# synsin0/StreamingFlow

Hardware: AMD Instinct MI355X
Metric: ODE-steps/s on 200x200x64 BEV (GRU-ODE future-state path, full FuturePredictionODE.forward) (higher is better)
Workload: dtype f32; 1 GPU; BASELINE config 2: C=64, BEV 200x200 (latent 50x50), timeset 'shipped' (8 observations, 7 targets), variable-step euler: 10 ODE steps + 8 jumps per sample, 32 sample(s) per forward per GPU; batch_per_gpu=32, parallelism=replicas x1 (sample sharding; no data-path collective)

## Files before the change

streamingflow_amd/csrc/conv_wino.hip:

```cpp
#include "sf_math.h"
#include "sf_launch.h"

#include <cstdlib>
#include <type_traits>

namespace sf {

#ifdef SF_STAMP
static __device__ unsigned long long* g_sf_stamps = nullptr;
hipError_t set_stamp_buffer_wino(unsigned long long* p) { return hipMemcpyToSymbol(HIP_SYMBOL(g_sf_stamps), &p, sizeof(p)); }
#else
hipError_t set_stamp_buffer_wino(unsigned long long*) { return hipErrorNotSupported; }
#endif

constexpr int WN_THREADS = 512;
constexpr long SF_WINO_SPLIT_WGS_DEFAULT = 512;
typedef __attribute__((address_space(3))) void wn_lds_void;

__device__ __forceinline__ f32x4 wn_lds_read128(const float* p) {
  typedef const __attribute__((address_space(3))) f32x4 lds_f4;
  return *(lds_f4*)p;
}
__device__ __forceinline__ void wn_barrier() {
  asm volatile("" ::: "memory");
// ... 139 lines not shown
  float* const Pbuf = Vbuf + G::NVB * G::V_FLOATS;
  float* const Park = Pbuf + G::NPB * G::P_FLOATS;
  float* const SBuf = Park + G::PARK;
  float* const SCbuf = SBuf + G::SB;
  float* const PVbuf = SCbuf + G::SC;
  (void)PVbuf;
  int lin_ = (int)blockIdx.x;
  const int pi_ = (int)__umulhi((unsigned)lin_, L.wn_m[0]);
  lin_ -= pi_ * L.wg_base[1];
  const ConvProblem& P = L.p[0];
  const ConvProblem& PX = L.p[pi_];
  const int tid = threadIdx.x, lane = tid & 63;
  const int wave = __builtin_amdgcn_readfirstlane(tid >> 6);
  const int H = P.Hout, W = P.Wout;
  const WnAxis ax(DIL ? W : 2, DIL ? P.dil : 1), ay(DIL ? H : 2, DIL ? P.dil : 1);
  const int tiles_x = DIL ? ax.nt : (W + 1) >> 1;
  const int tpi = tiles_x;
  const int nbx = ((CAT ? P.n_img * tiles_x : tiles_x) + TW - 1) / TW, nby = (L.wn_nty + TH - 1) / TH;
  const int ncb = P.cout_pad / COUT_T;
  const int nblk = nbx * nby * (CAT ? 1 : P.n_img), per_xcd = (nblk + 7) >> 3;
  const int lin = lin_, xcd = lin & 7, slot_ = lin >> 3;
#if SF_W5_MAGIC
  auto mdiv = [](const int nn, const unsigned m) { return m ? (int)__umulhi((unsigned)nn, m) : nn; };
  const unsigned m_ncb = L.wn_m[1], m_nbx = L.wn_m[2], m_nby = L.wn_m[3], m_tpi = L.wn_m[4];
  (void)m_tpi;
  const int tb_ = mdiv(slot_, m_ncb);
  int b = xcd * per_xcd + tb_;
  if (b >= nblk) return;
  const int bq_ = mdiv(b, m_nbx);
  const int bx = b - bq_ * nbx; b = bq_;
  const int bi_ = mdiv(b, m_nby);
  const int by = b - bi_ * nby;
  const int img = CAT ? mdiv(bx * TW, m_tpi) : bi_;
#else
  const int tb_ = slot_ / ncb;
  int b = xcd * per_xcd + tb_;
  if (b >= nblk) return;
  const int bx = b % nbx; b /= nbx;
  const int by = b % nby;
  const int img = CAT ? (bx * TW) / tpi : b / nby;
#endif
  const int ct0 = CAT ? bx * TW - img * tpi : 0;
  const int cn0 = CAT ? (tpi - ct0 < TW ? tpi - ct0 : TW) : TW;
  const int ty0 = L.wn_ty0 + by * TH, tx0 = CAT ? ct0 : bx * TW;
  int px0 = 0, pt0 = 0, py0 = 0, qt0 = 0;
  if constexpr (DIL) { ax.decode(tx0, px0, pt0); ay.decode(ty0, py0, qt0); }
  SF_STAMP_AT(L, 0);
#ifdef SF_STAMP
  SF_STAMP_VAL(L, 8, (unsigned long long)__builtin_amdgcn_s_getreg((31 << 11) | 4));
  SF_STAMP_VAL(L, 9, (unsigned long long)__builtin_amdgcn_s_getreg((31 << 11) | 20));
  SF_STAMP_VAL(L, 10, (unsigned long long)nkc_stamp(P));
#endif
  const int cout0 = (slot_ - tb_ * ncb) * COUT_T;
  const int nkc_g = P.cin_pad >> 4;
  const int nkc = GRP * nkc_g;
  const int NS = nkc * 4;
  const int c0 = P.c0;
  const int img_px_i = P.Hin * P.Win;
  const int up = DIL ? 0 : P.in_up;
  const int Win = P.Win;
#if defined(__HIP_DEVICE_COMPILE__)
  auto make_rsrc = [](const float* base, size_t bytes) {
    const unsigned nrec = bytes < 0x7fffffffull ? (unsigned)bytes : 0x7fffffffu;
    return __builtin_amdgcn_make_buffer_rsrc(const_cast<float*>(base), (short)0, (int)nrec, 0x00020000);
  };
  const size_t img_px = (size_t)P.Hin * P.Win;
  const size_t n_in = (CAT && img + 1 < P.n_img) ? 2 : 1;
  const __amdgpu_buffer_rsrc_t rsrc0 = make_rsrc(PX.in0 + (size_t)img * img_px * P.in0_cs, n_in * img_px * P.in0_cs * sizeof(float));
  const __amdgpu_buffer_rsrc_t rsrc1 = make_rsrc(PX.in1 ? PX.in1 + (size_t)img * img_px * P.in1_cs : PX.in0, PX.in1 ? n_in * img_px * P.in1_cs * sizeof(float) : 0);
  const __amdgpu_buffer_rsrc_t rsrc_u = make_rsrc(PX.w_wino, (size_t)nkc * 16 * P.cout_pad * 16 * sizeof(float));
#endif
  constexpr bool SCALED = G::SC > 0 && (EPI == EPI_AFFINE || EPI == EPI_SAMPLE);
  const bool scaled = SCALED && PX.in_scale != nullptr;
  typedef __attribute__((address_space(3))) int lds_int;
  float* const TabF = Park + 512;
  auto tab = [&](const int i) -> int { return *(const lds_int*)(TabF + i); };
  if constexpr (DIL) {
    if (tid < 72) {
      int v = 0;
      if (tid < PW) { int ix; v = ax.patch_coord(tid, px0, pt0, TW, W, ix) ? ix : -1; }
      else if (tid >= 32 && tid < 32 + G::PH) { int iy; v = ay.patch_coord(tid - 32, py0, qt0, TH, H, iy) ? iy : -1; }
      else if (tid >= 48 && tid < 60) {
        const bool isx = tid < 56;
        const int t = isx ? tx0 + (tid - 48) : ty0 + (tid - 56);
        const WnAxis& a = isx ? ax : ay;
        int pp, tt;
        a.decode(t, pp, tt);
        v = (t < a.nt && pp < P.dil) ? pp + P.dil * 2 * tt : (isx ? W : H);
      } else if (tid >= 60) {
        const bool isx = tid < 68;
        const int t = isx ? tx0 + (tid - 60) : ty0 + (tid - 68);
        int pp, tt;
        (isx ? ax : ay).decode(t, pp, tt);
        const int r = pp - (isx ? px0 : py0), lim = isx ? G::RX : G::RY;
        v = r < lim ? r : lim - 1;
      }
      *(lds_int*)(TabF + tid) = v;
    }
    asm volatile("s_waitcnt lgkmcnt(0)" ::: "memory");
    wn_barrier();
  }
  SF_STAMP_AT(L, 14);
  int pv0[NP], pv1[DIL ? 1 : NP];
  int piy[GRP > 1 ? NP : 1], pix_[GRP > 1 ? NP : 1];
  int pvs0[GRP > 1 ? NP : 1], pvs1[GRP > 1 ? NP : 1];
  (void)piy; (void)pix_; (void)pvs0; (void)pvs1;
  const int npw = G::ND / 8 + (wave < G::ND % 8 ? 1 : 0);
#pragma unroll
  for (int d = 0; d < NP; ++d) {
    const int e = (d * 8 + wave) * 64 + lane;
    const int pix = e >> 2, quad = e & 3;
    const int py = pix / PW, px = pix - py * PW;
    int iy = 2 * ty0 - 1 + py, ix = 2 * tx0 - 1 + px;
    int run = 0;
    if constexpr (CAT) {
      run = px >= 2 * cn0 + 2 ? 1 : 0;
      ix = run ? px - (2 * cn0 + 2) - 1 : ix;
    }
    bool ok = pix < G::NPX && (unsigned)iy < (unsigned)H && (unsigned)ix < (unsigned)W && (!CAT || (img + run < P.n_img && (run == 0 || cn0 < TW)));
    if constexpr (DIL) {
      const int pyc = py < G::PH ? py : 0;
      ix = tab(px); iy = tab(32 + pyc);
      ok = pix < G::NPX && ix >= 0 && iy >= 0;
    }
    const int pofs = DIL ? iy * W + ix : (iy >> up) * Win + (ix >> up) + (CAT ? run * img_px_i : 0);
    if constexpr (GRP > 1) {
      const bool in_blk = pix < G::NPX && (!CAT || (img + run < P.n_img && (run == 0 || cn0 < TW)));
      piy[d] = in_blk ? iy : -(1 << 20);
      pix_[d] = ix;
      pv0[d] = (pofs * P.in0_cs + quad * 4) * 4;
      pv1[d] = (pofs * P.in1_cs + quad * 4) * 4;
    } else {
      pv0[d] = ok ? (pofs * P.in0_cs + quad * 4) * 4 : (int)0x80000000;
      if constexpr (!DIL) pv1[d] = ok ? (pofs * P.in1_cs + quad * 4) * 4 : (int)0x80000000;
    }
  }
  int g_kc = 0, g_grp = 0;
  constexpr bool CAT_SC = CAT && G::PV == 0 && G::SC > 0;
  int run_bits = 0;
  if constexpr (CAT_SC) {
#pragma unroll
    for (int d = 0; d < NP; ++d) {
      const int pix = ((d * 8 + wave) * 64 + lane) >> 2;
      run_bits |= ((pix - (pix / PW) * PW) >= 2 * cn0 + 2 ? 1 : 0) << d;
    }
  }
  (void)run_bits;
  (void)g_kc; (void)g_grp;
  SF_STAMP_AT(L, 15);
  if constexpr (G::PV > 0) {
    static_assert(G::PV == 0 || NP == 1, "one piece per wave");
    *(lds_int*)(PVbuf + tid) = pv0[0];
    *(lds_int*)(PVbuf + 512 + tid) = pv1[0];
    asm volatile("s_waitcnt lgkmcnt(0)" ::: "memory");
  }
  auto issue_patch = [&](const int kc) {
    float* const dst = Pbuf + (G::NPB == 2 ? (kc & 1) : 0) * G::P_FLOATS;
    const bool from1 = !DIL && kc * 16 >= c0;
#if defined(__HIP_DEVICE_COMPILE__)
    if constexpr (GRP > 1) {
      if (g_kc == 0) {
        const int ga = (g_grp * 11) >> 5, gb = g_grp - 3 * ga;
        const int sy = 3 * ga - 3, sx = 3 * gb - 3;
        const int dlt = (sy * Win + sx) * 4;
#pragma unroll
        for (int d = 0; d < NP; ++d) {
          const bool okg = (unsigned)(piy[d] + sy) < (unsigned)H && (unsigned)(pix_[d] + sx) < (unsigned)W;
          pvs0[d] = okg ? pv0[d] + dlt * P.in0_cs : (int)0x80000000;
          pvs1[d] = okg ? pv1[d] + dlt * P.in1_cs : (int)0x80000000;
        }
      }
      const bool f1 = g_kc * 16 >= c0;
      const int so = f1 ? (g_kc * 16 - c0) * 4 : g_kc * 64;
#pragma unroll
      for (int d = 0; d < NP; ++d) {
        if (d >= npw) continue;
        float* const dB = dst + (d * 8 + wave) * 256;
        if (f1) {
          asm volatile("; patch from in1");
          __builtin_amdgcn_raw_ptr_buffer_load_lds(rsrc1, (wn_lds_void*)dB, 16, pvs1[d], so, 0, 0);
        } else {
          asm volatile("; patch from in0");
          __builtin_amdgcn_raw_ptr_buffer_load_lds(rsrc0, (wn_lds_void*)dB, 16, pvs0[d], so, 0, 0);
        }
      }
      if (++g_kc == nkc_g) { g_kc = 0; ++g_grp; }
      (void)kc; (void)from1;
      return;
    }
    if constexpr (G::PV > 0) {
      if (npw > 0) {
        int pv;
        asm volatile("ds_read_b32 %0, %1\n\ts_waitcnt lgkmcnt(0)" : "=v"(pv) : "v"((int)(size_t)(lds_int*)(PVbuf + (from1 ? 512 : 0) + tid)) : "memory");
        float* const dB = dst + wave * 256;
        if (from1) __builtin_amdgcn_raw_ptr_buffer_load_lds(rsrc1, (wn_lds_void*)dB, 16, pv, (kc * 16 - c0) * 4, 0, 0);
        else __builtin_amdgcn_raw_ptr_buffer_load_lds(rsrc0, (wn_lds_void*)dB, 16, pv, kc * 64, 0, 0);
      }
      return;
    }
#pragma unroll
    for (int d = 0; d < NP; ++d) {
      if (d >= npw) continue;
      float* const dB = dst + (d * 8 + wave) * 256;
      if constexpr (DIL) {
        __builtin_amdgcn_raw_ptr_buffer_load_lds(rsrc0, (wn_lds_void*)dB, 16, pv0[d], kc * 64, 0, 0);
      } else {
        if (from1) {
          asm volatile("; patch from in1");
          __builtin_amdgcn_raw_ptr_buffer_load_lds(rsrc1, (wn_lds_void*)dB, 16, pv1[d], (kc * 16 - c0) * 4, 0, 0);
        } else {
          asm volatile("; patch from in0");
          __builtin_amdgcn_raw_ptr_buffer_load_lds(rsrc0, (wn_lds_void*)dB, 16, pv0[d], kc * 64, 0, 0);
        }
      }
    }
#else
    (void)dst; (void)from1;
#endif
  };
  auto scale_patch = [&](const int kc) {
    if constexpr (SCALED) {
      if (scaled && kc * 16 < c0) {
// ... 45 lines not shown
                       : ((2 * tyl) * PW + 2 * txl + ((CAT && txl >= cn0) ? 2 : 0)) * 16 + quad * 4;
    const float* const a = src + tp + r1 * PW * 16;
    const float* const bb = src + tp + r2 * PW * 16;
    float* const o = dst + ((ih * 4) * WT + wt) * 16 + ((quad ^ ((wt >> 2) & 2)) << 2);
    typedef __attribute__((address_space(3))) f32x4 lds_f4w;
    const f32x4 w0 = wn_lds_read128(a) + sg * wn_lds_read128(bb);
    const f32x4 w2 = wn_lds_read128(a + 32) + sg * wn_lds_read128(bb + 32);
    *(lds_f4w*)(o) = wn5_sub4(w0, w2);
    const f32x4 w1 = wn_lds_read128(a + 16) + sg * wn_lds_read128(bb + 16);
    *(lds_f4w*)(o + WT * 16) = w1 + w2;
    *(lds_f4w*)(o + 2 * WT * 16) = wn5_sub4(w2, w1);
    const f32x4 w3 = wn_lds_read128(a + 48) + sg * wn_lds_read128(bb + 48);
    *(lds_f4w*)(o + 3 * WT * 16) = wn5_sub4(w1, w3);
  };
  float scv = 1.f;
  if constexpr (SCALED)
    if (scaled && tid < c0) scv = PX.in_scale[(size_t)img * c0 + tid];
    if (CAT_SC && scaled && tid >= c0 && tid < 2 * c0 && img + 1 < P.n_img) scv = PX.in_scale[(size_t)(img + 1) * c0 + (tid - c0)];
  issue_patch(0);
  f32x4 A[2][2];
  A[0][0] = load_A(0, 0); A[0][1] = load_A(0, 1);
  A[1][0] = load_A(1, 0); A[1][1] = load_A(1, 1);
  float sbv = tid < COUT_T ? 1.f : 0.f;
  if (tid < 2 * COUT_T) {
    const int co = cout0 + (tid < COUT_T ? tid : tid - COUT_T);
    if (co < P.cout) {
      if (tid < COUT_T) { if (PX.scale) sbv = PX.scale[co]; }
      else if (PX.bias) sbv = PX.bias[(P.bias_per_img ? (size_t)img * P.cout : 0) + co];
    }
  }
  SF_STAMP_AT(L, 11);
  wn_wait(4);
  if constexpr (SCALED) {
    if (scaled) {
      if (tid < G::SC) SCbuf[tid] = scv;
      asm volatile("s_waitcnt lgkmcnt(0)" ::: "memory");
      wn_barrier();
      scale_patch(0);
      asm volatile("s_waitcnt lgkmcnt(0)" ::: "memory");
    }
  }
  wn_barrier();
  SF_STAMP_AT(L, 12);
  transform(0);
  SF_STAMP_AT(L, 13);
  if (tid < 2 * COUT_T) SBuf[tid] = sbv;
  if (!MODE_A) issue_patch(1);
  asm volatile("s_waitcnt lgkmcnt(0)" ::: "memory");
  wn_barrier();
  SF_STAMP_AT(L, 1);

  f32x4 acc[4][2][NB];
  int b_cur = b_off;
  auto step = [&](const int kc, auto p_c, auto first_c) {
    constexpr int p = decltype(p_c)::value, slot = p & 1;
    constexpr bool first = decltype(first_c)::value;
    const float* const vb = Vbuf + (G::NVB == 2 ? (kc & 1) : 0) * G::V_FLOATS + p * WT * 16 + b_cur;
    f32x4 Bf[NB];
#pragma unroll
    for (int nb = 0; nb < NB; ++nb) Bf[nb] = wn_lds_read128(vb + nb * 256);
    __builtin_amdgcn_sched_barrier(0);
#pragma unroll
    for (int mb = 0; mb < 2; ++mb) {
#pragma unroll
      for (int e = 0; e < 4; ++e)
#pragma unroll
        for (int nb = 0; nb < NB; ++nb) {
          const f32x4 cin = (first && e == 0) ? (f32x4){0.f, 0.f, 0.f, 0.f} : acc[p][mb][nb];
          if (SF_W5_ABL & 16) acc[p][mb][nb] = (e == 0 && nb == 0 && mb == 0) ? cin + A[slot][mb] * Bf[nb] : cin;
          else acc[p][mb][nb] = __builtin_amdgcn_mfma_f32_16x16x4f32(A[slot][mb][e], Bf[nb][e], cin, 0, 0, 0);
        }
      __builtin_amdgcn_sched_barrier(0);
      if (!(SF_W5_ABL & 4)) A[slot][mb] = load_A(kc * 4 + p + 2, mb);
      __builtin_amdgcn_sched_barrier(0);
    }
  };
  auto chunk = [&](const int kc, auto first_c, auto more_c) {
    constexpr bool more = decltype(more_c)::value;
    if (MODE_A && more && !(SF_W5_ABL & 2)) issue_patch(kc + 1);
    step(kc, std::integral_constant<int, 0>{}, first_c);
    step(kc, std::integral_constant<int, 1>{}, first_c);
    if (MODE_A && more) {
      wn_wait(4);
      scale_patch(kc + 1);
      asm volatile("s_waitcnt lgkmcnt(0)" ::: "memory");
      if (!(SF_W5_ABL & 8)) wn_barrier();
      if (!(SF_W5_ABL & 1)) transform(kc + 1);
    }
    step(kc, std::integral_constant<int, 2>{}, first_c);
    step(kc, std::integral_constant<int, 3>{}, first_c);
    if (more) {
      if constexpr (MODE_A) {
        asm volatile("s_waitcnt lgkmcnt(0)" ::: "memory");
        if (!(SF_W5_ABL & 8)) wn_barrier();
      } else {
        wn_wait(4);
        wn_barrier();
        transform(kc + 1);
        if (kc + 2 < nkc) issue_patch(kc + 2);
        asm volatile("s_waitcnt lgkmcnt(0)" ::: "memory");
        wn_barrier();
      }
    }
  };
  chunk(0, std::true_type{}, std::true_type{});
  for (int kc = 1; kc + 1 < nkc; ++kc) chunk(kc, std::false_type{}, std::true_type{});
  if constexpr (WT == 16) {
    int t2 = tid;
    asm volatile("" : "+v"(t2));
    const int j2 = t2 & 15, g2 = (t2 & 63) >> 4;
    b_cur = (ih * 4 * WT + j2) * 16 + ((g2 ^ ((j2 >> 2) & 2)) << 2);
  }
  chunk(nkc - 1, std::false_type{}, std::false_type{});
  SF_STAMP_AT(L, 2);

  if (SF_W5_ABL & 32) {
    f32x4 sacc = (f32x4){0.f, 0.f, 0.f, 0.f};
#pragma unroll
    for (int p = 0; p < 4; ++p)
#pragma unroll
      for (int mb = 0; mb < 2; ++mb)
#pragma unroll
        for (int nb = 0; nb < NB; ++nb) sacc += acc[p][mb][nb];
    if (sacc[0] + sacc[1] + sacc[2] + sacc[3] == 1.2345f) PX.out[tid] = sacc[0];
    return;
  }
  float* const Tb = Vbuf;
  wn_barrier();
  int tid_e = tid;
  if constexpr (WT == 16) asm volatile("" : "+v"(tid_e));
  {
    typedef __attribute__((address_space(3))) f32x4 lds_f4w;
    const int j = tid_e & 15, g = (tid_e & 63) >> 4;
    const int tw_base = ((ih * 2) * WT + j) * 64;
#pragma unroll
    for (int mb = 0; mb < 2; ++mb) {
      const int tw = tw_base + (((hh * 8 + mb * 4 + g) ^ j) << 2);
#pragma unroll
      for (int nb = 0; nb < NB; ++nb) {
        const f32x4 m0 = acc[0][mb][nb], m1 = acc[1][mb][nb], m2 = acc[2][mb][nb], m3 = acc[3][mb][nb];
        *(lds_f4w*)(Tb + tw + nb * 16 * 64) = (m0 + m1) + m2;
        *(lds_f4w*)(Tb + tw + nb * 16 * 64 + WT * 64) = wn5_sub4(m1, m2 + m3);
      }
    }
  }
  const int cq = tid_e & 15, wt_e = WT == 32 ? tid_e >> 4 : (tid_e >> 4) & (WT - 1);
  const bool has_tile = WT == 32 || tid_e < 16 * WT;
  const int tyl_e = wt_e >> 3, txl_e = wt_e & 7;
  const bool run_e = CAT && txl_e >= cn0;
  const int ty = ty0 + tyl_e, tx = run_e ? txl_e - cn0 : tx0 + txl_e;
  int oy0 = 2 * ty, ox0 = 2 * tx, ostep = 1;
  if constexpr (DIL) {
    ostep = P.dil;
    ox0 = tab(48 + txl_e);
    oy0 = tab(56 + tyl_e);
  }
  constexpr bool affine = EPI == EPI_AFFINE, lng = EPI == EPI_LNG, smp = EPI == EPI_SAMPLE;
  const float* const t_a = (affine || lng) ? PX.add : PX.e0;
  const float* const t_b = PX.e1;
  const int cs_a = (affine || lng) ? P.add_cs : P.e0_cs, cs_b = P.e1_cs;
  const bool img_ok = has_tile && (!CAT || img + (run_e ? 1 : 0) < P.n_img);
  const bool x0 = img_ok && ox0 < W, x1 = img_ok && ox0 + ostep < W, y0ok = oy0 < H, y1ok = oy0 + ostep < H;
  const unsigned pix = (x0 && y0ok) ? (unsigned)(oy0 * W + ox0 + (run_e ? H * W : 0)) : 0u;
  const int cl = cq * 4;
  const int c = cout0 + cl;
  const bool c_ok = c < P.cout;
// ... 232 lines not shown
}
bool wino_takes(const ConvProblem& q, int epi) {
  if (epi == EPI_LNG) return wino_takes_ln7(q);
  if (epi == EPI_SAMPLE) {
    static const int on = [] { const char* v = std::getenv("SF_WINO_SAMPLE"); return v ? std::atoi(v) : 1; }();
    const double img_px = (double)q.Hin * q.Win;
    if (!on || q.dil != 1 || q.in_up || q.add || q.add_scale || q.pool2 || q.add_up || q.bias_per_img || q.scale || (q.cout % 8) || (q.c1 != 0) ||
        2.0 * 4.0 * img_px * q.cout >= 2147483648.0 || (!q.e0 && !q.philox))
      return false;
    return wino_takes(q, EPI_AFFINE);
  }
  if (epi != EPI_AFFINE && epi != EPI_BLEND) return false;
  if (!q.w_wino || q.KH != 3 || q.KW != 3 || q.stride != 1 || q.dil < 1 || q.pad != q.dil || (q.in_up && q.dil != 1) || q.gather || q.gate || q.se_sum ||
      (q.in_scale && (epi != EPI_AFFINE || q.dil != 1 || q.c0 > 256)) ||
      q.nsplit > 1 || q.chansum || q.acc_in || q.fuse_w || q.out_planar || (epi == EPI_AFFINE && (q.mode & 4)))
    return false;
  if (q.pool2 && (epi != EPI_AFFINE || q.dil != 1 || q.out2 || (q.Hout & 1) || (q.Wout & 1))) return false;
  if (q.add_up && (epi != EPI_AFFINE || q.dil != 1 || !q.add || (q.Hout & 1) || (q.Wout & 1))) return false;
  if ((q.c0 % 16) || (q.c1 % 16) || q.c0 + q.c1 != q.cin_pad || (q.cout_pad % 64) || (q.cout % 4)) return false;
  if (q.Hout != (q.Hin << q.in_up) || q.Wout != (q.Win << q.in_up) || q.Hout < 16 || q.Wout < 32) return false;
  if (q.dil > 1 && (q.c1 != 0 || epi != EPI_AFFINE || q.Hout / q.dil < 5 || q.Wout / q.dil < 5)) return false;
  const double img_bytes = 4.0 * q.Hin * q.Win;
  if (img_bytes * q.out_cs >= 2147483648.0 || img_bytes * q.add_cs >= 2147483648.0 || img_bytes * q.e0_cs >= 2147483648.0 ||
      img_bytes * q.e1_cs >= 2147483648.0 || img_bytes * q.out2_cs >= 2147483648.0)
    return false;
  if (img_bytes * q.in0_cs >= 2147483648.0 || img_bytes * q.in1_cs >= 2147483648.0 || 4.0 * 16 * q.cout_pad * q.cin_pad >= 2147483648.0) return false;
  return true;
}

static bool wino_cat(const ConvProblem& q) {
  static const int on = [] { const char* v = std::getenv("SF_WINO_CAT"); return v ? std::atoi(v) : 1; }();
  const int tpi = (q.Wout + 1) / 2;
  static const int cat_scaled = [] { const char* v = std::getenv("SF_WINO_CAT_SCALED"); return v ? std::atoi(v) : 1; }();
  if (!on || q.dil != 1 || q.in_up || q.n_img < 2 || tpi < 8 || q.bias_per_img || ((q.in_scale || q.add_scale) && !cat_scaled)) return false;
  const int plain = (tpi + 7) / 8 * 8;
  if (plain * 100 < tpi * 110) {
    if (q.cout_pad < 128 || plain * 100 < tpi * 104) return false;
    const char* const v = std::getenv("SF_WINO_CAT_WIDE");
    if (v && std::atoi(v) == 0) return false;
  }
  const double img_bytes = 4.0 * q.Hin * q.Win;
  const int cs = q.in0_cs > q.in1_cs ? q.in0_cs : q.in1_cs;
  const int co = q.out_cs > q.add_cs ? q.out_cs : q.add_cs;
  const int ce = q.e0_cs > q.e1_cs ? q.e0_cs : q.e1_cs;
  const int cm = co > ce ? (co > q.out2_cs ? co : q.out2_cs) : (ce > q.out2_cs ? ce : q.out2_cs);
  return 2.0 * img_bytes * cs < 2147483648.0 && 2.0 * img_bytes * cm < 2147483648.0;
}
int wino_variant(const ConvProblem& q) {
  if (q.cout_pad % 64) return -1;
  if (q.dil > 1) return 3;
  if (wino_cat(q)) return 4;
  return 2;
}
double wino_tiles(const ConvProblem& q) {
  if (q.dil > 1) return (double)q.n_img * WnAxis(q.Hout, q.dil).nt * WnAxis(q.Wout, q.dil).nt;
  return (double)q.n_img * ((q.Hout + 1) / 2) * ((q.Wout + 1) / 2);
}
static long wino5_wgs(const ConvLaunch& L, bool cat, int rows, int th) {
  const ConvProblem& P = L.p[0];
  const int tiles_x = (P.Wout + 1) / 2;
  const long nby = (rows + th - 1) / th;
  const long blocks = cat ? nby * (((long)P.n_img * tiles_x + 7) / 8) : (long)P.n_img * nby * ((tiles_x + 7) / 8);
  return ((blocks + 7) / 8) * 8 * (P.cout_pad / 64) * L.nprob;
}
template <int EPI, bool DIL = false, bool CAT = false, int TH_ = 4, int GRP = 1>
static hipError_t launch_wino5_t(const ConvLaunch& L, hipStream_t stream, const int row0 = 0, const int rows = -1) {
  typedef Wino5Geo<DIL, CAT, TH_> G;
  auto kern = conv_wino5_kernel<EPI, DIL, CAT, TH_, GRP>;
  constexpr int lds = G::LDS_FLOATS * 4;
  static bool attr_done[64] = {};
  int dev = 0;
  if (hipGetDevice(&dev) != hipSuccess || dev < 0 || dev >= 64) return hipErrorInvalidDevice;
  if (!attr_done[dev]) {
    hipError_t e = hipFuncSetAttribute(reinterpret_cast<const void*>(kern), hipFuncAttributeMaxDynamicSharedMemorySize, lds);
    if (e != hipSuccess) return e;
    attr_done[dev] = true;
  }
  const ConvProblem& P = L.p[0];
  const int tiles_x = DIL ? WnAxis(P.Wout, P.dil).nt : (P.Wout + 1) / 2, tiles_all = DIL ? WnAxis(P.Hout, P.dil).nt : (P.Hout + 1) / 2;
  const int tiles_y = rows < 0 ? tiles_all : rows;
  if (row0 < 0 || tiles_y < 1 || row0 + tiles_y > tiles_all || (DIL && tiles_y != tiles_all) || (row0 + tiles_y < tiles_all && tiles_y % G::TH)) return hipErrorInvalidValue;
  const long blocks = CAT ? (long)((tiles_y + G::TH - 1) / G::TH) * (((long)P.n_img * tiles_x + G::TW - 1) / G::TW)
                          : (long)P.n_img * ((tiles_y + G::TH - 1) / G::TH) * ((tiles_x + G::TW - 1) / G::TW);
  const long grid1 = ((blocks + 7) / 8) * 8 * (P.cout_pad / G::COUT_T), grid = grid1 * L.nprob;
  if (grid > 0x7fffffffL) return hipErrorInvalidValue;
  ConvLaunch L2 = L;
  L2.wg_base[0] = 0;
  L2.wg_base[1] = (int)grid1;
  L2.wn_ty0 = row0; L2.wn_nty = tiles_y;
  const long nbx = ((CAT ? (long)P.n_img * tiles_x : tiles_x) + G::TW - 1) / G::TW, nby = (tiles_y + G::TH - 1) / G::TH, ncb = P.cout_pad / G::COUT_T;
  if ((grid1 / 8 + 1) * ncb >= 0x100000000L || (blocks + 8) * nbx >= 0x100000000L || (blocks + 8) * nby >= 0x100000000L ||
      (nbx * G::TW + G::TW) * tiles_x >= 0x100000000L)
    return hipErrorInvalidValue;
  if (L.nprob > 1 && grid * grid1 >= 0x100000000L) return hipErrorInvalidValue;
  L2.wn_m[0] = L.nprob > 1 ? magic(grid1) : 1u;
  L2.wn_m[1] = magic(ncb); L2.wn_m[2] = magic(nbx); L2.wn_m[3] = magic(nby); L2.wn_m[4] = magic(tiles_x);
  hipLaunchKernelGGL(kern, dim3((unsigned)grid, 1, 1), dim3(WN_THREADS), lds, stream, L2);
  return hipGetLastError();
}
bool wino_same_geometry(const ConvProblem& a, const ConvProblem& b) {
  return a.n_img == b.n_img && a.Hin == b.Hin && a.Win == b.Win && a.Hout == b.Hout && a.Wout == b.Wout && a.in_up == b.in_up && a.dil == b.dil &&
         a.c0 == b.c0 && a.c1 == b.c1 && a.cin_pad == b.cin_pad && a.cout == b.cout && a.cout_pad == b.cout_pad &&
         (a.in_scale != nullptr) == (b.in_scale != nullptr) && (a.in1 != nullptr) == (b.in1 != nullptr) && (a.add != nullptr) == (b.add != nullptr) &&
         (a.add_scale != nullptr) == (b.add_scale != nullptr) && (a.out2 != nullptr) == (b.out2 != nullptr) && (a.scale != nullptr) == (b.scale != nullptr) &&
         (a.bias != nullptr) == (b.bias != nullptr) && a.in0_cs == b.in0_cs && a.in1_cs == b.in1_cs && a.add_cs == b.add_cs && a.out_cs == b.out_cs &&
         a.out_co == b.out_co && a.out2_cs == b.out2_cs && a.e0_cs == b.e0_cs && a.e1_cs == b.e1_cs && a.act == b.act && a.mode == b.mode &&
         a.gate_from == b.gate_from && a.clamp_from == b.clamp_from && a.clamp_lo == b.clamp_lo && a.clamp_hi == b.clamp_hi &&
         a.bias_per_img == b.bias_per_img && a.pool2 == b.pool2 && a.add_up == b.add_up && wino_variant(a) == wino_variant(b);
}
hipError_t launch_conv_wino(const ConvLaunch& L, int epi, hipStream_t stream) {
  if (L.nprob < 1 || L.nprob > SF_MAX_GROUP) return hipErrorInvalidValue;
  for (int i = 0; i < L.nprob; ++i)
    if (!wino_takes(L.p[i], epi) || !wino_same_geometry(L.p[0], L.p[i])) return hipErrorInvalidValue;
  const bool affine = epi == EPI_AFFINE;
  const int var = wino_variant(L.p[0]);
  if (epi == EPI_SAMPLE) {
    if (var == 2) return launch_wino5_t<EPI_SAMPLE>(L, stream);
    if (var == 4) return launch_wino5_t<EPI_SAMPLE, false, true>(L, stream);
    return hipErrorInvalidValue;
  }
  if (epi == EPI_LNG) {
    if (var == 2) return launch_wino5_t<EPI_LNG, false, false, 4, 9>(L, stream);
    if (var == 4) return launch_wino5_t<EPI_LNG, false, true, 4, 9>(L, stream);
    return hipErrorInvalidValue;
  }
  static const long small_wgs = [] { const char* v = std::getenv("SF_WINO_SMALL_WGS"); return v ? std::atol(v) : 1000L; }();
  if (var == 3) return affine ? launch_wino5_t<EPI_AFFINE, true>(L, stream) : hipErrorInvalidValue;
  if (var != 2 && var != 4) return hipErrorInvalidValue;
  const bool cat = var == 4;
  const bool only32 = cat && L.p[0].in_scale;
  auto launch = [&](const bool small, const int row0, const int rows) -> hipError_t {
    if (cat) {
      if (small) return affine ? launch_wino5_t<EPI_AFFINE, false, true, 2>(L, stream, row0, rows) : launch_wino5_t<EPI_BLEND, false, true, 2>(L, stream, row0, rows);
      return affine ? launch_wino5_t<EPI_AFFINE, false, true>(L, stream, row0, rows) : launch_wino5_t<EPI_BLEND, false, true>(L, stream, row0, rows);
    }
    if (small) return affine ? launch_wino5_t<EPI_AFFINE, false, false, 2>(L, stream, row0, rows) : launch_wino5_t<EPI_BLEND, false, false, 2>(L, stream, row0, rows);
    return affine ? launch_wino5_t<EPI_AFFINE>(L, stream, row0, rows) : launch_wino5_t<EPI_BLEND>(L, stream, row0, rows);
  };
  const int tiles_y = (L.p[0].Hout + 1) / 2;
  const bool small = !only32 && wino5_wgs(L, cat, tiles_y, 4) < small_wgs;
  const char* const sv = std::getenv("SF_WINO_SPLIT_WGS");
  const long split_wgs = sv ? std::atol(sv) : SF_WINO_SPLIT_WGS_DEFAULT;
  const int main_rows = tiles_y & ~3, rem_rows = tiles_y - main_rows;
  if (!small && !only32 && split_wgs > 0 && rem_rows > 0 && main_rows > 0 && wino5_wgs(L, cat, rem_rows, 2) >= split_wgs) {
    const hipError_t e = launch(wino5_wgs(L, cat, main_rows, 4) < small_wgs, 0, main_rows);
    return e != hipSuccess ? e : launch(true, main_rows, rem_rows);
  }
  return launch(small, 0, -1);
}

}
```

streamingflow_amd/csrc/dispatch.hip:

```cpp
#include "dispatch.h"

#include <cstdio>
#include <cstdlib>
#include <cstring>
#include <vector>

namespace {

__global__ void zero_fill_kernel(float4* __restrict__ p, size_t n4) {
  for (size_t i = (size_t)blockIdx.x * blockDim.x + threadIdx.x; i < n4; i += (size_t)gridDim.x * blockDim.x)
    p[i] = make_float4(0.f, 0.f, 0.f, 0.f);
}
__global__ void copy_kernel(const float4* __restrict__ src, float4* __restrict__ dst, size_t n4) {
  for (size_t i = (size_t)blockIdx.x * blockDim.x + threadIdx.x; i < n4; i += (size_t)gridDim.x * blockDim.x) dst[i] = src[i];
}
__global__ void flow_poison_kernel(const unsigned* __restrict__ err, float* __restrict__ a, size_t na, float* __restrict__ b, size_t nb) {
  if (__builtin_nontemporal_load(err) == 0) return;
  const float q = __builtin_nanf("");
  for (size_t i = (size_t)blockIdx.x * blockDim.x + threadIdx.x; i < na + nb; i += (size_t)gridDim.x * blockDim.x) {
    if (i < na) a[i] = q;
    else b[i - na] = q;
  }
}

// ... 299 lines not shown
  if (!A.ok()) return;
  g_seg = fb = new FlowBuilder(table, done, done + FLOW_DONE_COUNTERS, st);
  if (zero_fill(done, (FLOW_DONE_COUNTERS + 64) * sizeof(unsigned), st) != hipSuccess) status = SF_ERR_LAUNCH;
}
FlowScope::~FlowScope() {
  if (fb) g_seg = nullptr;
  delete fb;
}
const unsigned* FlowScope::err() const { return fb ? fb->err : nullptr; }
int flow_copy_out(const float* src, float* dst, size_t n, hipStream_t st) {
  if (g_seg && g_seg->add_copy(src, dst, n) == SF_OK) return SF_OK;
  SF_TRY(seg_flush());
  SF_HIP(copy_floats(src, dst, n, st));
  return SF_OK;
}
int flow_close(const unsigned* err, float* a, size_t na, float* b, size_t nb, hipStream_t st) {
  if (err) {
    hipLaunchKernelGGL(flow_poison_kernel, dim3(256), dim3(256), 0, st, err, a, na, b, nb);
    SF_HIP(hipGetLastError());
  }
  g_flow_err_last = err;
  return SF_OK;
}
int set_flow_mode(int on) {
  const int was = g_flow_mode < 0 ? tune().persist : g_flow_mode;
  g_flow_mode = on < 0 ? -1 : (on ? 1 : 0);
  return was;
}
int flow_errors(hipStream_t st) {
  if (!g_flow_err_last) return SF_ERR_INVALID;
  unsigned v = 0;
  if (hipMemcpyAsync(&v, g_flow_err_last, sizeof(v), hipMemcpyDeviceToHost, st) != hipSuccess) return SF_ERR_LAUNCH;
  if (hipStreamSynchronize(st) != hipSuccess) return SF_ERR_LAUNCH;
  return (int)(v > 0x3fffffffu ? 0x3fffffffu : v);
}

static Cost direct_cost(int key, const ConvProblem* ps, int n) {
  Cost c{key, 0, 0};
  for (int i = 0; i < n; ++i) {
    const ConvProblem& q = ps[i];
    const double Pi = (double)q.n_img * q.Hout * q.Wout;
    const double K = (double)q.KH * q.KW * (q.c0 + q.c1);
    c.flops += 2.0 * Pi * q.cout * K;
    c.bytes += 4.0 * ((double)q.n_img * q.Hin * q.Win * (q.c0 + q.c1) + (double)q.cout * K + Pi * q.cout);
  }
  return c;
}
static Cost wino_cost(const ConvProblem* ps, int n, int epi) {
  const int wv = wino_variant(ps[0]);
  Cost c{(16 + (wv == 4 ? 2 : wv)) * 8 + epi, 0, 0};
  for (int i = 0; i < n; ++i) {
    const ConvProblem& q = ps[i];
    const double grp = q.KH == 7 ? 9.0 : 1.0;
    c.flops += 2.0 * 16.0 * grp * wino_tiles(q) * q.cout * (q.c0 + q.c1);
    c.bytes += 4.0 * ((double)q.n_img * q.Hin * q.Win * (q.c0 + q.c1) + 16.0 * grp * q.cout * (q.c0 + q.c1) + (double)q.n_img * q.Hout * q.Wout * q.cout);
  }
  return c;
}
static void select_bf16x3(ConvLaunch& L) {
  if (!tune().b3) return;
  bool all3 = true;
  for (int i = 0; i < L.nprob; ++i) all3 = all3 && L.p[i].w3 != nullptr;
  for (int i = 0; i < L.nprob; ++i) L.p[i].use_w3 = all3 ? 1 : 0;
}

constexpr int NOT_MINE = 1;

static int run_wide_ln(ConvLaunch& L, int epi, hipStream_t st) {
  SF_TRY(seg_flush());
  for (int i = 0; i < L.nprob; ++i) {
    const ConvProblem& q = L.p[i];
    if (q.gate || q.gather || q.in_scale || q.se_sum || !one_source_per_chunk(q) || !offsets_fit32(q, 256.0)) return SF_ERR_UNSUPPORTED;
  }
  select_bf16x3(L);
  SF_HIP(timed([&] { return launch_conv_glds(L, epi, 5, 0, st); }, [&] { return direct_cost(5 * 8 + epi, L.p, L.nprob); }, st));
  return SF_OK;
}

static int wino_list_launch(const ConvLaunch& W1, int epi, hipStream_t st) {
  const ConvProblem& q = W1.p[0];
  hipEvent_t a, b;
  SF_HIP(hipEventCreate(&a)); SF_HIP(hipEventCreate(&b));
  SF_HIP(hipEventRecord(a, st));
  SF_HIP(launch_conv_wino(W1, epi, st));
  SF_HIP(hipEventRecord(b, st));
  SF_HIP(hipEventSynchronize(b));
  float ms = 0.f;
  SF_HIP(hipEventElapsedTime(&ms, a, b));
  (void)hipEventDestroy(a); (void)hipEventDestroy(b);
  std::fprintf(stderr, "[sf-wino] n=%d %dx%d c=%d+%d->%d epi=%d act=%d mode=%d add=%d add_scale=%d out2=%d in_scale=%d bias_img=%d clamp=%d dil=%d up=%d var=%d us=%.1f gflop=%.3f\n",
               q.n_img, q.Hout, q.Wout, q.c0, q.c1, q.cout, epi, q.act, q.mode, q.add != nullptr, q.add_scale != nullptr, q.out2 != nullptr,
               q.in_scale != nullptr, q.bias_per_img, q.clamp_from >= 0, q.dil, q.in_up, wino_variant(q), ms * 1e3,
               2.0 * 16.0 * wino_tiles(q) * q.cout * (q.c0 + q.c1) * 1e-9);
  return SF_OK;
}
static void wino_why(const ConvProblem* ps, int n, int epi) {
  for (int i = 0; i < n; ++i)
    if (ps[i].KH == 3 && !wino_takes(ps[i], epi))
      std::fprintf(stderr, "[sf] direct 3x3: n=%d/%d %dx%d c=%d+%d->%d stride=%d dil=%d up=%d gather=%d gate=%d in_scale=%d se_sum=%d nsplit=%d chansum=%d acc_in=%d fuse=%d mode=%d wino=%d\n",
                   i, n, ps[i].Hout, ps[i].Wout, ps[i].c0, ps[i].c1, ps[i].cout, ps[i].stride, ps[i].dil, ps[i].in_up, ps[i].gather != nullptr,
                   ps[i].gate != nullptr, ps[i].in_scale != nullptr, ps[i].se_sum != nullptr, ps[i].nsplit, ps[i].chansum != nullptr,
                   ps[i].acc_in != nullptr, ps[i].fuse_w != nullptr, ps[i].mode, ps[i].w_wino != nullptr);
}
static int run_wino(const ConvProblem* ps, int n, int P, int epi, hipStream_t st) {
  if (!tune().wino || P < tune().wino_min_p || !(epi == EPI_AFFINE || epi == EPI_BLEND || epi == EPI_LNG || epi == EPI_SAMPLE)) return NOT_MINE;
  bool takes[SF_MAX_GROUP];
  int n_wino = 0;
// ... 328 lines not shown
```

streamingflow_amd/csrc/sf_launch.h:

```cpp
#pragma once
#include "sf_device.h"

namespace sf {
hipError_t launch_conv(const ConvLaunch& L, int epi, int cfg, hipStream_t stream);
hipError_t launch_conv_direct(const ConvLaunch& L, int epi, int mt, int ks, hipStream_t stream);
hipError_t launch_conv_glds(const ConvLaunch& L, int epi, int tile, int variant, hipStream_t stream);
hipError_t set_stamp_buffer(unsigned long long* p);
int glds_occupancy(int which);
hipError_t set_stamp_buffer_sp(unsigned long long* p);
hipError_t set_stamp_buffer_wino(unsigned long long* p);
hipError_t launch_conv_sp(const ConvLaunch& L, int epi, bool scaled, int bn, hipStream_t stream);
hipError_t launch_conv_wino(const ConvLaunch& L, int epi, hipStream_t stream);
bool wino_takes(const ConvProblem& q, int epi);
bool wino_same_geometry(const ConvProblem& a, const ConvProblem& b);
int wino_variant(const ConvProblem& q);
double wino_tiles(const ConvProblem& q);
hipError_t launch_sp_flow(const SpFlow& F, int grid, bool b3, hipStream_t stream);
hipError_t launch_flow_write(const void* host_src, void* dev_dst, size_t bytes, hipStream_t stream);
bool sp_flow_has(int epi, bool scaled, int bn);
int sp_flow_capacity(bool b3);
hipError_t launch_convnext_mlp(const float* t, const float* x, float* out, const float* w1, const float* s1, const float* b1, const float* w2, const float* s2, const float* b2, long P, hipStream_t stream);
hipError_t launch_transpose(const float* in, float* out, int n, int rows, int cols, hipStream_t s);
hipError_t launch_transpose_strided(const float* in, float* out, int n, int rows, int cols, size_t in_stride, size_t out_stride, hipStream_t s);
hipError_t launch_maxpool2(const float* in, float* out, int n, int Hin, int Win, int C, int ceil_pad, hipStream_t s);
hipError_t launch_mean_from_partials(const float* part, float* out, int n, int nslab, int C, int hw, hipStream_t s);
hipError_t launch_logsigmoid(const float* in, float* out, size_t n, hipStream_t s);
hipError_t launch_upsample2(const float* in, float* out, int n, int Hin, int Win, int C, hipStream_t s);
hipError_t launch_broadcast_channels(const float* vec, float* out, int n, int HW, int k, int out_cs, int out_co, hipStream_t s);
hipError_t launch_upsample_bilinear2_add(const float* in, const float* skip, float* out, int n, int Hin, int Win, int C, hipStream_t s);
hipError_t launch_se_fc(const float* chansum, int ntile, int C, int Cr, int hw, const float* fc0, const float* fc2, float* scale, int n_img, hipStream_t s);
hipError_t launch_chan_partial(const float* in, float* part, int n, int HW, int C, int nslab, hipStream_t s);
hipError_t launch_dwconv7_ln(const float* in, float* out, const float* wdw, const float* bdw, const float* lnw, const float* lnb, int n, int H, int W, int C, float eps, hipStream_t s);
hipError_t launch_aspp_pool(const float* in, float* part, float* bias_img, int n, int HW, int C, int hid, const float* w1, const float* s1, const float* b1, const float* wp, const float* ps, const float* pb, int nslab, hipStream_t s);

inline unsigned magic(long d) { return d <= 1 ? 0u : (unsigned)((0x100000000ull + (unsigned long long)d - 1) / (unsigned long long)d); }
}
```

Before: 2150 ODE-steps/s.

## Skip structurally-zero Winograd sub-products in 7x7 grouped conv; allow batching across K geometry

For 7x7 convolutions decomposed into nine 3x3 Winograd groups, the third group row/column reaches past the 7x7 kernel. The kernel now omits the MFMA step on the Winograd products that are all zero there, and adjusts A-fragment prefetch offsets to match. This is on by default and can be turned off with SF_WINO_LN7_SKIP. Per-problem channel strides are now read from the extended per-problem params, so problems with different input channel layouts can share one grouped launch. The cost is more fragile loop bookkeeping, with a risk of wrong indexing if the zero pattern assumption fails.

```diff
diff --git a/streamingflow_amd/csrc/conv_wino.hip b/streamingflow_amd/csrc/conv_wino.hip
--- a/streamingflow_amd/csrc/conv_wino.hip
+++ b/streamingflow_amd/csrc/conv_wino.hip
@@ -215,10 +215,11 @@
   SF_STAMP_VAL(L, 10, (unsigned long long)nkc_stamp(P));
 #endif
   const int cout0 = (slot_ - tb_ * ncb) * COUT_T;
-  const int nkc_g = P.cin_pad >> 4;
+  const int nkc_g = PX.cin_pad >> 4;
   const int nkc = GRP * nkc_g;
   const int NS = nkc * 4;
-  const int c0 = P.c0;
+  const int c0 = PX.c0;
+  const int in0_cs = PX.in0_cs, in1_cs = PX.in1_cs;
   const int img_px_i = P.Hin * P.Win;
   const int up = DIL ? 0 : P.in_up;
   const int Win = P.Win;
@@ -229,8 +230,8 @@
   };
   const size_t img_px = (size_t)P.Hin * P.Win;
   const size_t n_in = (CAT && img + 1 < P.n_img) ? 2 : 1;
-  const __amdgpu_buffer_rsrc_t rsrc0 = make_rsrc(PX.in0 + (size_t)img * img_px * P.in0_cs, n_in * img_px * P.in0_cs * sizeof(float));
-  const __amdgpu_buffer_rsrc_t rsrc1 = make_rsrc(PX.in1 ? PX.in1 + (size_t)img * img_px * P.in1_cs : PX.in0, PX.in1 ? n_in * img_px * P.in1_cs * sizeof(float) : 0);
+  const __amdgpu_buffer_rsrc_t rsrc0 = make_rsrc(PX.in0 + (size_t)img * img_px * in0_cs, n_in * img_px * in0_cs * sizeof(float));
+  const __amdgpu_buffer_rsrc_t rsrc1 = make_rsrc(PX.in1 ? PX.in1 + (size_t)img * img_px * in1_cs : PX.in0, PX.in1 ? n_in * img_px * in1_cs * sizeof(float) : 0);
   const __amdgpu_buffer_rsrc_t rsrc_u = make_rsrc(PX.w_wino, (size_t)nkc * 16 * P.cout_pad * 16 * sizeof(float));
 #endif
   constexpr bool SCALED = G::SC > 0 && (EPI == EPI_AFFINE || EPI == EPI_SAMPLE);
@@ -291,11 +292,11 @@
       const bool in_blk = pix < G::NPX && (!CAT || (img + run < P.n_img && (run == 0 || cn0 < TW)));
       piy[d] = in_blk ? iy : -(1 << 20);
       pix_[d] = ix;
-      pv0[d] = (pofs * P.in0_cs + quad * 4) * 4;
-      pv1[d] = (pofs * P.in1_cs + quad * 4) * 4;
+      pv0[d] = (pofs * in0_cs + quad * 4) * 4;
+      pv1[d] = (pofs * in1_cs + quad * 4) * 4;
     } else {
-      pv0[d] = ok ? (pofs * P.in0_cs + quad * 4) * 4 : (int)0x80000000;
-      if constexpr (!DIL) pv1[d] = ok ? (pofs * P.in1_cs + quad * 4) * 4 : (int)0x80000000;
+      pv0[d] = ok ? (pofs * in0_cs + quad * 4) * 4 : (int)0x80000000;
+      if constexpr (!DIL) pv1[d] = ok ? (pofs * in1_cs + quad * 4) * 4 : (int)0x80000000;
     }
   }
   int g_kc = 0, g_grp = 0;
@@ -329,8 +330,8 @@
 #pragma unroll
         for (int d = 0; d < NP; ++d) {
           const bool okg = (unsigned)(piy[d] + sy) < (unsigned)H && (unsigned)(pix_[d] + sx) < (unsigned)W;
-          pvs0[d] = okg ? pv0[d] + dlt * P.in0_cs : (int)0x80000000;
-          pvs1[d] = okg ? pv1[d] + dlt * P.in1_cs : (int)0x80000000;
+          pvs0[d] = okg ? pv0[d] + dlt * in0_cs : (int)0x80000000;
+          pvs1[d] = okg ? pv1[d] + dlt * in1_cs : (int)0x80000000;
         }
       }
       const bool f1 = g_kc * 16 >= c0;
@@ -482,8 +483,11 @@
 
   f32x4 acc[4][2][NB];
   int b_cur = b_off;
-  auto step = [&](const int kc, auto p_c, auto first_c) {
+  const bool ln7_skip = GRP > 1 && L.wn_m[5] != 0;
+  (void)ln7_skip;
+  auto step = [&](const int kc, auto p_c, auto first_c, auto skip_c) {
     constexpr int p = decltype(p_c)::value, slot = p & 1;
+    constexpr bool skip3 = decltype(skip_c)::value;
     constexpr bool first = decltype(first_c)::value;
     const float* const vb = Vbuf + (G::NVB == 2 ? (kc & 1) : 0) * G::V_FLOATS + p * WT * 16 + b_cur;
     f32x4 Bf[NB];
@@ -501,15 +505,16 @@
           else acc[p][mb][nb] = __builtin_amdgcn_mfma_f32_16x16x4f32(A[slot][mb][e], Bf[nb][e], cin, 0, 0, 0);
         }
       __builtin_amdgcn_sched_barrier(0);
-      if (!(SF_W5_ABL & 4)) A[slot][mb] = load_A(kc * 4 + p + 2, mb);
+      if (!(SF_W5_ABL & 4)) A[slot][mb] = load_A(kc * 4 + p + ((GRP > 1 && p == 1 && skip3) ? 4 : 2), mb);
       __builtin_amdgcn_sched_barrier(0);
     }
   };
-  auto chunk = [&](const int kc, auto first_c, auto more_c) {
+  auto chunk = [&](const int kc, auto first_c, auto more_c, auto skip_c) {
     constexpr bool more = decltype(more_c)::value;
+    constexpr bool skip3 = GRP > 1 && decltype(skip_c)::value;
     if (MODE_A && more && !(SF_W5_ABL & 2)) issue_patch(kc + 1);
-    step(kc, std::integral_constant<int, 0>{}, first_c);
-    step(kc, std::integral_constant<int, 1>{}, first_c);
+    step(kc, std::integral_constant<int, 0>{}, first_c, std::false_type{});
+    step(kc, std::integral_constant<int, 1>{}, first_c, skip_c);
     if (MODE_A && more) {
       wn_wait(4);
       scale_patch(kc + 1);
@@ -517,8 +522,8 @@
       if (!(SF_W5_ABL & 8)) wn_barrier();
       if (!(SF_W5_ABL & 1)) transform(kc + 1);
     }
-    step(kc, std::integral_constant<int, 2>{}, first_c);
-    step(kc, std::integral_constant<int, 3>{}, first_c);
+    step(kc, std::integral_constant<int, 2>{}, first_c, std::false_type{});
+    if constexpr (!skip3) step(kc, std::integral_constant<int, 3>{}, first_c, std::false_type{});
     if (more) {
       if constexpr (MODE_A) {
         asm volatile("s_waitcnt lgkmcnt(0)" ::: "memory");
@@ -533,15 +538,26 @@
       }
     }
   };
-  chunk(0, std::true_type{}, std::true_type{});
-  for (int kc = 1; kc + 1 < nkc; ++kc) chunk(kc, std::false_type{}, std::true_type{});
+  chunk(0, std::true_type{}, std::true_type{}, std::false_type{});
+  if constexpr (GRP > 1) {
+    int kc = 1;
+    for (int ga = 0; ga < 3; ++ga) {
+      const int n_full = (ln7_skip ? 2 : 3) * nkc_g, n_skip = ln7_skip ? nkc_g : 0;
+      for (const int end = ga * 3 * nkc_g + n_full - (ga == 2 && !ln7_skip ? 1 : 0); kc < end; ++kc) chunk(kc, std::false_type{}, std::true_type{}, std::false_type{});
+      for (const int end = ga * 3 * nkc_g + n_full + n_skip - (ga == 2 ? 1 : 0); kc < end; ++kc) chunk(kc, std::false_type{}, std::true_type{}, std::true_type{});
+    }
+  } else {
+    for (int kc = 1; kc + 1 < nkc; ++kc) chunk(kc, std::false_type{}, std::true_type{}, std::false_type{});
+  }
   if constexpr (WT == 16) {
     int t2 = tid;
     asm volatile("" : "+v"(t2));
     const int j2 = t2 & 15, g2 = (t2 & 63) >> 4;
     b_cur = (ih * 4 * WT + j2) * 16 + ((g2 ^ ((j2 >> 2) & 2)) << 2);
   }
-  chunk(nkc - 1, std::false_type{}, std::false_type{});
+  chunk(nkc - 1, std::false_type{}, std::false_type{}, std::integral_constant<bool, (GRP > 1)>{});
+  if constexpr (GRP > 1)
+    if (!ln7_skip) step(nkc - 1, std::integral_constant<int, 3>{}, std::false_type{}, std::false_type{});
   SF_STAMP_AT(L, 2);
 
   if (SF_W5_ABL & 32) {
@@ -880,6 +896,10 @@
   if (wino_cat(q)) return 4;
   return 2;
 }
+bool wino_ln7_skip() {
+  const char* const v = std::getenv("SF_WINO_LN7_SKIP");
+  return !v || std::atoi(v) != 0;
+}
 double wino_tiles(const ConvProblem& q) {
   if (q.dil > 1) return (double)q.n_img * WnAxis(q.Hout, q.dil).nt * WnAxis(q.Wout, q.dil).nt;
   return (double)q.n_img * ((q.Hout + 1) / 2) * ((q.Wout + 1) / 2);
@@ -923,15 +943,20 @@
   if (L.nprob > 1 && grid * grid1 >= 0x100000000L) return hipErrorInvalidValue;
   L2.wn_m[0] = L.nprob > 1 ? magic(grid1) : 1u;
   L2.wn_m[1] = magic(ncb); L2.wn_m[2] = magic(nbx); L2.wn_m[3] = magic(nby); L2.wn_m[4] = magic(tiles_x);
+  L2.wn_m[5] = (GRP > 1 && wino_ln7_skip()) ? 1u : 0u;
   hipLaunchKernelGGL(kern, dim3((unsigned)grid, 1, 1), dim3(WN_THREADS), lds, stream, L2);
   return hipGetLastError();
 }
 bool wino_same_geometry(const ConvProblem& a, const ConvProblem& b) {
+  const char* const gk = std::getenv("SF_WINO_GROUP_K");
+  const bool same_k = a.c0 == b.c0 && a.c1 == b.c1 && a.cin_pad == b.cin_pad && (a.in1 != nullptr) == (b.in1 != nullptr) && a.in0_cs == b.in0_cs &&
+                      a.in1_cs == b.in1_cs;
+  if (!same_k && ((gk && std::atoi(gk) == 0) || a.KH != b.KH)) return false;
   return a.n_img == b.n_img && a.Hin == b.Hin && a.Win == b.Win && a.Hout == b.Hout && a.Wout == b.Wout && a.in_up == b.in_up && a.dil == b.dil &&
-         a.c0 == b.c0 && a.c1 == b.c1 && a.cin_pad == b.cin_pad && a.cout == b.cout && a.cout_pad == b.cout_pad &&
-         (a.in_scale != nullptr) == (b.in_scale != nullptr) && (a.in1 != nullptr) == (b.in1 != nullptr) && (a.add != nullptr) == (b.add != nullptr) &&
+         a.cout == b.cout && a.cout_pad == b.cout_pad &&
+         (a.in_scale != nullptr) == (b.in_scale != nullptr) && (a.add != nullptr) == (b.add != nullptr) &&
          (a.add_scale != nullptr) == (b.add_scale != nullptr) && (a.out2 != nullptr) == (b.out2 != nullptr) && (a.scale != nullptr) == (b.scale != nullptr) &&
-         (a.bias != nullptr) == (b.bias != nullptr) && a.in0_cs == b.in0_cs && a.in1_cs == b.in1_cs && a.add_cs == b.add_cs && a.out_cs == b.out_cs &&
+         (a.bias != nullptr) == (b.bias != nullptr) && a.add_cs == b.add_cs && a.out_cs == b.out_cs &&
          a.out_co == b.out_co && a.out2_cs == b.out2_cs && a.e0_cs == b.e0_cs && a.e1_cs == b.e1_cs && a.act == b.act && a.mode == b.mode &&
          a.gate_from == b.gate_from && a.clamp_from == b.clamp_from && a.clamp_lo == b.clamp_lo && a.clamp_hi == b.clamp_hi &&
          a.bias_per_img == b.bias_per_img && a.pool2 == b.pool2 && a.add_up == b.add_up && wino_variant(a) == wino_variant(b);
diff --git a/streamingflow_amd/csrc/dispatch.hip b/streamingflow_amd/csrc/dispatch.hip
--- a/streamingflow_amd/csrc/dispatch.hip
+++ b/streamingflow_amd/csrc/dispatch.hip
@@ -375,7 +375,8 @@
   for (int i = 0; i < n; ++i) {
     const ConvProblem& q = ps[i];
     const double grp = q.KH == 7 ? 9.0 : 1.0;
-    c.flops += 2.0 * 16.0 * grp * wino_tiles(q) * q.cout * (q.c0 + q.c1);
+    const double prods = (q.KH == 7 && wino_ln7_skip()) ? 16.0 * 9.0 - 3.0 * 4.0 : 16.0 * grp;
+    c.flops += 2.0 * prods * wino_tiles(q) * q.cout * (q.c0 + q.c1);
     c.bytes += 4.0 * ((double)q.n_img * q.Hin * q.Win * (q.c0 + q.c1) + 16.0 * grp * q.cout * (q.c0 + q.c1) + (double)q.n_img * q.Hout * q.Wout * q.cout);
   }
   return c;
diff --git a/streamingflow_amd/csrc/sf_launch.h b/streamingflow_amd/csrc/sf_launch.h
--- a/streamingflow_amd/csrc/sf_launch.h
+++ b/streamingflow_amd/csrc/sf_launch.h
@@ -13,6 +13,7 @@
 hipError_t launch_conv_wino(const ConvLaunch& L, int epi, hipStream_t stream);
 bool wino_takes(const ConvProblem& q, int epi);
 bool wino_same_geometry(const ConvProblem& a, const ConvProblem& b);
+bool wino_ln7_skip();
 int wino_variant(const ConvProblem& q);
 double wino_tiles(const ConvProblem& q);
 hipError_t launch_sp_flow(const SpFlow& F, int grid, bool b3, hipStream_t stream);
```

Result: no change. 2164 ODE-steps/s (median of 6 runs) (+0.6%).
